# Teque5/caf_cookoff

Hardware: NVIDIA B200
Metric: CAF cells/s (400x8192 fp64 surface + peak) (higher is better)
Workload: dtype f64

## Files before the change

### caf_cookoff_b200/csrc/caf_kernels.cuh

```cuda
#pragma once
#include <cstdint>
#include <type_traits>
#include "fft16.cuh"

namespace caf {

constexpr int kThreads = 512;
constexpr int kL0 = 4096;
constexpr int kM = 8192;

enum Mode : int {
    kSurface = 0,
    kSpectrumHalf = 1,
    kSpectrumFull = 2,
    kXcorFull = 3,
    kXcorHalf = 4
};

struct PeakOut {
    double value;
    double freq_hz;
    unsigned long long doppler_idx;
    unsigned long long delay_idx;
};

template <typename T>
struct RowArgs {
    const cx<T>* in;
    const cx<T>* in2;
    cx<T>* hperm;
    const double* freqs;
    void* out;
    T* row_peak_val;
    unsigned long long* row_peak_idx;
    PeakOut* peak;
    unsigned long long* peak_words;
    unsigned long long row_offset;
    unsigned int* peak_seq;
    unsigned int seq_val;
    unsigned int* done_counter;
    unsigned int done_last;
    const cx<T>* tw1;
    const cx<T>* tw2;
    const cx<T>* g;
    double dt;
    int L;
    int D;
    int P;
    cx<T>* hshare;
    unsigned int* hflag;
    unsigned int epoch;
    int hprod1;
    const uint4* pull_src;
    uint4* pull_dst;
    unsigned int pull_n16;
    unsigned int* pull_counter;
    unsigned int pull_target;
    unsigned int flags;
    long long* trace;
};

template <typename T> struct Fab;
template <> struct Fab<double> {
    using E = double;
    static constexpr int kRegion = 280;
    static constexpr int kPlane = 16 * kRegion;
    static constexpr int kPipe = 2 * kPlane;
    static __device__ __forceinline__ void st(E* p, int i, double2 v) { p[i] = v.x; p[kPlane + i] = v.y; }
    static __device__ __forceinline__ double2 ld(const E* p, int i) { return make_double2(p[i], p[kPlane + i]); }
};
template <> struct Fab<float> {
    using E = float2;
    static constexpr int kRegion = 256;
    static constexpr int kPipe = 16 * kRegion;
    static __device__ __forceinline__ void st(E* p, int i, float2 v) { p[i] = v; }
    static __device__ __forceinline__ float2 ld(const E* p, int i) { return p[i]; }
};

template <typename T>
struct SmemLayout {
    static constexpr size_t kS = sizeof(typename Fab<T>::E) * 2 * Fab<T>::kPipe;
    static constexpr size_t kPtab = sizeof(cx<T>) * 2 * 2 * 48;
    static constexpr size_t kRed = 16 * 8 + 16 * 8;
    static constexpr size_t kCand = 2 * 256 * (8 + 4);
    static constexpr size_t kMisc = 64;
    static constexpr size_t kNeedle = sizeof(T) * 2 * kL0;
    static constexpr size_t offPtab = kS, offRed = offPtab + kPtab, offCand = offRed + kRed, offMisc = offCand + kCand,
                            offNeedle = offMisc + kMisc;
    static constexpr size_t kTotalNoNeedle = offNeedle;
    static constexpr size_t kTotal = offNeedle + kNeedle;
};

template <typename T>
struct Ctx {
    static constexpr bool kPadded = std::is_same<T, double>::value;
    typename Fab<T>::E* Sr;
    cx<T>* ptab;
    uint32_t tm_A;
    uint32_t tm_B;
    uint32_t tm_g;
    int w, lane, r, h, t;
    int wb;
    int hs[2];
    int hr;
    long long* tr;

    __device__ __forceinline__ void init(unsigned char* smem_raw, int tid) {
        const int hw_warp = tid >> 5;
        lane = tid & 31; r = tid >> 8;
        h = (lane & 7) | ((lane >> 1) & 8);
        const int sub = (lane >> 3) & 1;
        w = 2 * (hw_warp & 7) + sub;
        t = 16 * w + h;
        wb = Fab<T>::kRegion * w;
        hs[0] = h ^ (sub << 3); hs[1] = hs[0] ^ 8;
        hr = h ^ (((sub ^ h) & 1) << 3);
        Sr = reinterpret_cast<typename Fab<T>::E*>(smem_raw) + r * Fab<T>::kPipe;
        ptab = nullptr; tm_A = tm_B = tm_g = 0; tr = nullptr;
    }
    __device__ __forceinline__ int ix_block(int k) const {
        if constexpr (kPadded) return k * Fab<T>::kRegion + (t ^ ((t & 16) >> 1));
        else return k * 256 + 16 * w + hs[k & 1];
    }
    __device__ __forceinline__ int ix_own(int i) const {
        if constexpr (kPadded) return wb + 16 * i + (h ^ ((i & 1) << 3));
        else return wb + 16 * i + hs[i & 1];
    }
    __device__ __forceinline__ int ix_tw(int k) const {
        if constexpr (kPadded) return wb + 17 * k + h;
        else return wb + 16 * k + (hs[k & 1] ^ k);
    }
    __device__ __forceinline__ int ix_tr(int m) const {
        if constexpr (kPadded) return wb + 17 * h + m;
        else return wb + 16 * h + (m ^ hr);
    }
};

#ifdef CAF_TRACE
#define CAF_TR(c_, slot_) do { if ((c_).tr && (c_).lane == 0) (c_).tr[slot_] = clock64(); } while (0)
#else
#define CAF_TR(c_, slot_) do { } while (0)
#endif

__device__ __forceinline__ void tmem_ld_x16(uint32_t taddr, uint32_t (&r)[16]) {
    asm volatile("tcgen05.ld.sync.aligned.32x32b.x16.b32 {%0,%1,%2,%3,%4,%5,%6,%7,%8,%9,%10,%11,%12,%13,%14,%15}, [%16];\n"
                 : "=r"(r[0]), "=r"(r[1]), "=r"(r[2]), "=r"(r[3]), "=r"(r[4]), "=r"(r[5]), "=r"(r[6]), "=r"(r[7]),
                   "=r"(r[8]), "=r"(r[9]), "=r"(r[10]), "=r"(r[11]), "=r"(r[12]), "=r"(r[13]), "=r"(r[14]), "=r"(r[15])
                 : "r"(taddr) : "memory");
}
__device__ __forceinline__ void tmem_st_x16(uint32_t taddr, const uint32_t (&r)[16]) {
    asm volatile("tcgen05.st.sync.aligned.32x32b.x16.b32 [%0], {%1,%2,%3,%4,%5,%6,%7,%8,%9,%10,%11,%12,%13,%14,%15,%16};\n"
                 :: "r"(taddr), "r"(r[0]), "r"(r[1]), "r"(r[2]), "r"(r[3]), "r"(r[4]), "r"(r[5]), "r"(r[6]), "r"(r[7]),
                    "r"(r[8]), "r"(r[9]), "r"(r[10]), "r"(r[11]), "r"(r[12]), "r"(r[13]), "r"(r[14]), "r"(r[15]) : "memory");
}
__device__ __forceinline__ void tmem_ld_x8(uint32_t taddr, uint32_t (&r)[8]) {
    asm volatile("tcgen05.ld.sync.aligned.32x32b.x8.b32 {%0,%1,%2,%3,%4,%5,%6,%7}, [%8];\n"
                 : "=r"(r[0]), "=r"(r[1]), "=r"(r[2]), "=r"(r[3]), "=r"(r[4]), "=r"(r[5]), "=r"(r[6]), "=r"(r[7])
                 : "r"(taddr) : "memory");
}
__device__ __forceinline__ void tmem_st_x8(uint32_t taddr, const uint32_t (&r)[8]) {
    asm volatile("tcgen05.st.sync.aligned.32x32b.x8.b32 [%0], {%1,%2,%3,%4,%5,%6,%7,%8};\n"
                 :: "r"(taddr), "r"(r[0]), "r"(r[1]), "r"(r[2]), "r"(r[3]), "r"(r[4]), "r"(r[5]), "r"(r[6]), "r"(r[7]) : "memory");
}
__device__ __forceinline__ void tmem_wait_ld() { asm volatile("tcgen05.wait::ld.sync.aligned;\n" ::: "memory"); }
__device__ __forceinline__ void tmem_wait_st() { asm volatile("tcgen05.wait::st.sync.aligned;\n" ::: "memory"); }

__device__ __forceinline__ void tmem_ld_x4(uint32_t taddr, uint32_t (&r)[4]) {
    asm volatile("tcgen05.ld.sync.aligned.32x32b.x4.b32 {%0,%1,%2,%3}, [%4];\n"
                 : "=r"(r[0]), "=r"(r[1]), "=r"(r[2]), "=r"(r[3]) : "r"(taddr) : "memory");
}
__device__ __forceinline__ void tmem_st_x4(uint32_t taddr, const uint32_t (&r)[4]) {
    asm volatile("tcgen05.st.sync.aligned.32x32b.x4.b32 [%0], {%1,%2,%3,%4};\n"
                 :: "r"(taddr), "r"(r[0]), "r"(r[1]), "r"(r[2]), "r"(r[3]) : "memory");
}
__device__ __forceinline__ void tmem_ld_x2(uint32_t taddr, uint32_t (&r)[2]) {
    asm volatile("tcgen05.ld.sync.aligned.32x32b.x2.b32 {%0,%1}, [%2];\n" : "=r"(r[0]), "=r"(r[1]) : "r"(taddr) : "memory");
}
__device__ __forceinline__ void tmem_st_x2(uint32_t taddr, const uint32_t (&r)[2]) {
    asm volatile("tcgen05.st.sync.aligned.32x32b.x2.b32 [%0], {%1,%2};\n" :: "r"(taddr), "r"(r[0]), "r"(r[1]) : "memory");
}

template <typename T> struct TmemGeom;
template <> struct TmemGeom<double> { static constexpr int kColsPerC = 4, kAlloc = 512; };
template <> struct TmemGeom<float>  { static constexpr int kColsPerC = 2, kAlloc = 256; };

struct Raw4d { uint32_t r[16]; };
struct Raw4f { uint32_t r[8]; };
template <typename T> struct raw4_of;
template <> struct raw4_of<double> { using type = Raw4d; };
template <> struct raw4_of<float>  { using type = Raw4f; };
__device__ __forceinline__ void tmem_ld4_issue(uint32_t taddr, Raw4d& q) { tmem_ld_x16(taddr, q.r); }
__device__ __forceinline__ void tmem_ld4_issue(uint32_t taddr, Raw4f& q) { tmem_ld_x8(taddr, q.r); }
__device__ __forceinline__ void tmem_unpack4(const Raw4d& q, double2 (&o)[4]) {
#pragma unroll
    for (int i = 0; i < 4; ++i) {
        o[i].x = __hiloint2double((int)q.r[4 * i + 1], (int)q.r[4 * i]);
        o[i].y = __hiloint2double((int)q.r[4 * i + 3], (int)q.r[4 * i + 2]);
    }
}
__device__ __forceinline__ void tmem_unpack4(const Raw4f& q, float2 (&o)[4]) {
#pragma unroll
    for (int i = 0; i < 4; ++i) { o[i].x = __uint_as_float(q.r[2 * i]); o[i].y = __uint_as_float(q.r[2 * i + 1]); }
}
__device__ __forceinline__ void tmem_st4(uint32_t taddr, const double2 (&v)[4]) {
    uint32_t r[16];
#pragma unroll
    for (int i = 0; i < 4; ++i) {
        r[4 * i] = (uint32_t)__double2loint(v[i].x); r[4 * i + 1] = (uint32_t)__double2hiint(v[i].x);
        r[4 * i + 2] = (uint32_t)__double2loint(v[i].y); r[4 * i + 3] = (uint32_t)__double2hiint(v[i].y);
    }
    tmem_st_x16(taddr, r);
}
__device__ __forceinline__ void tmem_st4(uint32_t taddr, const float2 (&v)[4]) {
    uint32_t r[8];
#pragma unroll
    for (int i = 0; i < 4; ++i) { r[2 * i] = __float_as_uint(v[i].x); r[2 * i + 1] = __float_as_uint(v[i].y); }
    tmem_st_x8(taddr, r);
}

__device__ __forceinline__ double2 tmem_ld1(uint32_t taddr, double) {
    uint32_t r[4];
    tmem_ld_x4(taddr, r);
    tmem_wait_ld();
    return make_double2(__hiloint2double((int)r[1], (int)r[0]), __hiloint2double((int)r[3], (int)r[2]));
}
__device__ __forceinline__ float2 tmem_ld1(uint32_t taddr, float) {
    uint32_t r[2];
    tmem_ld_x2(taddr, r);
    tmem_wait_ld();
    return make_float2(__uint_as_float(r[0]), __uint_as_float(r[1]));
}
__device__ __forceinline__ void tmem_st1(uint32_t taddr, double2 v) {
    uint32_t r[4] = {(uint32_t)__double2loint(v.x), (uint32_t)__double2hiint(v.x), (uint32_t)__double2loint(v.y), (uint32_t)__double2hiint(v.y)};
    tmem_st_x4(taddr, r);
}
__device__ __forceinline__ void tmem_st1(uint32_t taddr, float2 v) {
    uint32_t r[2] = {__float_as_uint(v.x), __float_as_uint(v.y)};
    tmem_st_x2(taddr, r);
}

template <typename T>
__device__ __forceinline__ cx<T> ldg(const cx<T>* p) { return __ldg(p); }

__device__ __forceinline__ double2 unit_phasor(double n, double phi, double exact_sub) {
    double hi = n * phi;
    double lo = fma(n, phi, -hi);
    double fr = (hi - rint(hi)) + lo - exact_sub;
    fr -= rint(fr);
    double s, c;
    sincospi(2.0 * fr, &s, &c);
    return make_double2(c, s);
}

__device__ __forceinline__ void bar_group(int r) { asm volatile("bar.sync %0, 256;\n" :: "r"(r + 1) : "memory"); }

__device__ __forceinline__ void mbar_init(uint64_t* mb, int count) {
    asm volatile("mbarrier.init.shared::cta.b64 [%0], %1;\n" :: "r"((uint32_t)__cvta_generic_to_shared(mb)), "r"(count) : "memory");
}
__device__ __forceinline__ void mbar_arrive(uint64_t* mb) {
    asm volatile("{\n.reg .b64 st;\nmbarrier.arrive.shared::cta.b64 st, [%0];\n}\n"
                 :: "r"((uint32_t)__cvta_generic_to_shared(mb)) : "memory");
}
__device__ __forceinline__ void mbar_wait(uint64_t* mb, int parity) {
    const uint32_t addr = (uint32_t)__cvta_generic_to_shared(mb);
    asm volatile("{\n.reg .pred p;\nWAIT_%=:\nmbarrier.try_wait.parity.shared::cta.b64 p, [%0], %1;\n@p bra DONE_%=;\nbra WAIT_%=;\nDONE_%=:\n}\n"
                 :: "r"(addr), "r"(parity) : "memory");
}

template <typename T>
__device__ __forceinline__ void tmem_store_power_table(uint32_t taddr, cx<T> w) {
    constexpr int kC = TmemGeom<T>::kColsPerC;
    const cx<T> w2 = csq(w), w4 = csq(w2);
    cx<T> q[4];
    q[0] = mk<T>((T)1, (T)0); q[1] = w4; q[2] = csq(w4); q[3] = cmul(q[2], w4);
    tmem_st4(taddr, q);
    q[0] = w; q[1] = cmul(q[0], w4); q[2] = cmul(q[1], w4); q[3] = cmul(q[2], w4);
    tmem_st4(taddr + 4 * kC, q);
    q[0] = w2; q[1] = cmul(q[0], w4); q[2] = cmul(q[1], w4); q[3] = cmul(q[2], w4);
    tmem_st4(taddr + 8 * kC, q);
    q[0] = cmul(w2, w); q[1] = cmul(q[0], w4); q[2] = cmul(q[1], w4); q[3] = cmul(q[2], w4);
    tmem_st4(taddr + 12 * kC, q);
}

template <typename T, bool INV, int MODE, bool Q0_ONE>
__device__ __forceinline__ void fft16_in_tmem(cx<T> (&v)[16], uint32_t taddr) {
    constexpr int kC = TmemGeom<T>::kColsPerC;
    typename raw4_of<T>::type r0, r1, r2, r3;
    cx<T> q[4];
    tmem_ld4_issue(taddr, r0);
    tmem_wait_ld();
    tmem_ld4_issue(taddr + 4 * kC, r1);
    tmem_unpack4(r0, q);
    radix4_in<T, INV, MODE, Q0_ONE>(v[0], v[4], v[8], v[12], q[0], q[1], q[2], q[3]);
    tmem_wait_ld();
    tmem_ld4_issue(taddr + 8 * kC, r2);
    tmem_unpack4(r1, q);
    radix4_in<T, INV, MODE, false>(v[1], v[5], v[9], v[13], q[0], q[1], q[2], q[3]);
    tmem_wait_ld();
    tmem_ld4_issue(taddr + 12 * kC, r3);
    tmem_unpack4(r2, q);
    radix4_in<T, INV, MODE, false>(v[2], v[6], v[10], v[14], q[0], q[1], q[2], q[3]);
    tmem_wait_ld();
    tmem_unpack4(r3, q);
    radix4_in<T, INV, MODE, false>(v[3], v[7], v[11], v[15], q[0], q[1], q[2], q[3]);
    fft16_stage_b<T, INV>(v);
}

template <typename T, int MODE>
__device__ __forceinline__ void mul_table_tmem(cx<T> (&v)[16], uint32_t taddr) {
    constexpr int kC = TmemGeom<T>::kColsPerC;
    typename raw4_of<T>::type r0, r1, r2, r3;
    cx<T> q[4];
    tmem_ld4_issue(taddr, r0);
    tmem_ld4_issue(taddr + 4 * kC, r1);
    tmem_wait_ld();
    tmem_ld4_issue(taddr + 8 * kC, r2);
    tmem_ld4_issue(taddr + 12 * kC, r3);
    tmem_unpack4(r0, q);
#pragma unroll
    for (int a = 1; a < 4; ++a) v[4 * a] = tw_apply<MODE>(v[4 * a], q[a]);
    tmem_unpack4(r1, q);
#pragma unroll
    for (int a = 0; a < 4; ++a) v[1 + 4 * a] = tw_apply<MODE>(v[1 + 4 * a], q[a]);
    tmem_wait_ld();
    tmem_unpack4(r2, q);
#pragma unroll
    for (int a = 0; a < 4; ++a) v[2 + 4 * a] = tw_apply<MODE>(v[2 + 4 * a], q[a]);
    tmem_unpack4(r3, q);
#pragma unroll
    for (int a = 0; a < 4; ++a) v[3 + 4 * a] = tw_apply<MODE>(v[3 + 4 * a], q[a]);
}

template <typename T, typename Hook, typename Hook3>
__device__ __forceinline__ void forward_tail(cx<T> (&v)[16], const Ctx<T>& c,
                                             uint64_t* empty_mb, int empty_parity, Hook&& hook, Hook3&& hook3) {
    mul_table_tmem<T, kTwMul>(v, c.tm_A);
    CAF_TR(c, 3);
    if (empty_mb) mbar_wait(empty_mb, empty_parity);
    hook();
    bar_group(c.r);
#pragma unroll
    for (int k = 0; k < 16; ++k) Fab<T>::st(c.Sr, c.ix_block(k), v[k]);
    CAF_TR(c, 4);
    bar_group(c.r);
#pragma unroll
    for (int i = 0; i < 16; ++i) v[i] = Fab<T>::ld(c.Sr, c.ix_own(i));
    CAF_TR(c, 5);

    fft16<T, false>(v);
    CAF_TR(c, 6);
    __syncwarp();
#pragma unroll
    for (int k = 0; k < 16; ++k) Fab<T>::st(c.Sr, c.ix_tw(k), v[k]);
    __syncwarp();
#pragma unroll
    for (int m = 0; m < 16; ++m) v[m] = Fab<T>::ld(c.Sr, c.ix_tr(m));
    hook3();
    CAF_TR(c, 7);

    fft16_in_tmem<T, false, kTwMul, true>(v, c.tm_B);
    CAF_TR(c, 8);
}
template <typename T, typename Hook, typename Hook3>
__device__ __forceinline__ void forward_4096(cx<T> (&v)[16], const Ctx<T>& c,
                                             uint64_t* empty_mb, int empty_parity, Hook&& hook, Hook3&& hook3) {
    fft16<T, false>(v);
    forward_tail<T>(v, c, empty_mb, empty_parity, hook, hook3);
}

template <typename T, bool HFUSED>
__device__ __forceinline__ void inverse_4096(cx<T> (&v)[16], const Ctx<T>& c, uint32_t tm_h) {
    if constexpr (HFUSED) fft16_in_tmem<T, true, kTwConjX, false>(v, tm_h);
    else fft16<T, true>(v);
    CAF_TR(c, 10);
    __syncwarp();
#pragma unroll
    for (int k = 0; k < 16; ++k) Fab<T>::st(c.Sr, c.ix_tw(k), v[k]);
    __syncwarp();
#pragma unroll
    for (int m = 0; m < 16; ++m) v[m] = Fab<T>::ld(c.Sr, c.ix_tr(m));
    CAF_TR(c, 11);

    fft16_in_tmem<T, true, kTwMulConj, true>(v, c.tm_B);
    CAF_TR(c, 12);
    __syncwarp();
#pragma unroll
    for (int k = 0; k < 16; ++k) Fab<T>::st(c.Sr, c.ix_own(k), v[k]);
    CAF_TR(c, 13);
    bar_group(c.r);
#pragma unroll
    for (int k = 0; k < 16; ++k) v[k] = Fab<T>::ld(c.Sr, c.ix_block(k));
    CAF_TR(c, 14);

    fft16_in_tmem<T, true, kTwMulConj, true>(v, c.tm_A);
    CAF_TR(c, 15);
}

template <typename T, int J>
__device__ __forceinline__ cx<T> mul_w32_inv(cx<T> a) {
    constexpr T Cc[8] = {(T)1.0L, (T)0.98078528040323044913L, (T)0.92387953251128675613L, (T)0.83146961230254523708L,
                         (T)0.70710678118654752440L, (T)0.55557023301960222474L, (T)0.38268343236508977173L,
                         (T)0.19509032201612826785L};
    constexpr T Ss[8] = {(T)0.0L, (T)0.19509032201612826785L, (T)0.38268343236508977173L, (T)0.55557023301960222474L,
                         (T)0.70710678118654752440L, (T)0.83146961230254523708L, (T)0.92387953251128675613L,
                         (T)0.98078528040323044913L};
    if constexpr (J == 0) return a;
    else if constexpr (J == 8) return mk<T>(-a.y, a.x);
    else if constexpr (J < 8) return mk<T>(a.x * Cc[J] - a.y * Ss[J], a.x * Ss[J] + a.y * Cc[J]);
    else return mk<T>(-a.x * Ss[J - 8] - a.y * Cc[J - 8], a.x * Cc[J - 8] - a.y * Ss[J - 8]);
}

__device__ __forceinline__ void pack_peak_words(const PeakOut& p, unsigned long long global_row_offset,
                                                unsigned long long* __restrict__ words) {
    words[0] = (unsigned long long)__double_as_longlong(p.value);
    words[1] = (p.doppler_idx == ~0ull) ? ~0ull : p.doppler_idx + global_row_offset;
    words[2] = p.delay_idx;
    words[3] = (unsigned long long)__double_as_longlong(p.freq_hz);
}

template <typename T>
__device__ __forceinline__ void amax_take(T& best, int& bidx, T m, int k) {
    if (m > best || (m == best && k < bidx)) { best = m; bidx = k; }
}

template <int I> using ic = std::integral_constant<int, I>;

template <typename T, int MODE, bool FULL, bool SHARED = false>
__global__ void __launch_bounds__(kThreads, 1) caf_rows_kernel(const RowArgs<T> a) {
    using C = cx<T>;
    using SL = SmemLayout<T>;
    using TG = TmemGeom<T>;
    extern __shared__ __align__(16) unsigned char smem_raw[];
    C* ptab = reinterpret_cast<C*>(smem_raw + SL::offPtab);
    unsigned long long* red_idx = reinterpret_cast<unsigned long long*>(smem_raw + SL::offRed);
    double* red_val = reinterpret_cast<double*>(smem_raw + SL::offRed + 128);
    double* cand_val = reinterpret_cast<double*>(smem_raw + SL::offCand);
    int* cand_idx = reinterpret_cast<int*>(smem_raw + SL::offCand + 2 * 256 * 8);
    uint32_t* misc = reinterpret_cast<uint32_t*>(smem_raw + SL::offMisc);
    uint64_t* mb_full = reinterpret_cast<uint64_t*>(smem_raw + SL::offMisc + 16);
    uint64_t* mb_empty = reinterpret_cast<uint64_t*>(smem_raw + SL::offMisc + 24);

    const int tid = threadIdx.x;
#ifdef CAF_TRACE
    long long tr_g0 = 0, tr_c0 = clock64();
    asm volatile("mov.u64 %0, %%globaltimer;" : "=l"(tr_g0));
#endif
    Ctx<T> c;
    const int hw_warp = tid >> 5;
    c.init(smem_raw, tid);
    c.ptab = ptab;
    const int w = c.w, lane = c.lane, r = c.r, h = c.h, t = c.t, tg = tid & 255, wg = hw_warp & 7;

    constexpr bool kHalfZero = (MODE == kSurface || MODE == kSpectrumHalf || MODE == kXcorHalf);
    constexpr bool kWritesH = (MODE == kSpectrumHalf || MODE == kSpectrumFull);
    constexpr bool kUseTmem = (MODE == kSurface);
    T* const ndl_re = reinterpret_cast<T*>(smem_raw + SL::offNeedle);
    T* const ndl_im = ndl_re + kL0;

    const int rows_per_pair = (MODE == kSurface) ? a.D : 1;
    const long long n_items = (long long)a.P * rows_per_pair;
    const int lo = (int)(n_items * blockIdx.x / gridDim.x), hi = (int)(n_items * (blockIdx.x + 1) / gridDim.x);
    int pair = lo / rows_per_pair, row = lo - pair * rows_per_pair;

    int buf = 0;
    int cur_pair = -1;
    int posts = 0;
    bool drain_pending = false;
    bool h_from_share = false;
    C v[16];

    if constexpr (MODE == kSurface) asm volatile("griddepcontrol.launch_dependents;\n" ::: "memory");
    const C tb0 = ldg<T>(a.tw1 + 256 + t), tb1 = ldg<T>(a.tw2 + 16 + h), tb4 = ldg<T>(a.g + t);
    bool preloaded = false;
    double phi_first = 0.0;
    if constexpr (MODE == kSurface) {
        if (lo < hi) {
            const bool producer0 = !SHARED || (int)blockIdx.x == ((r == 0) ? 0 : a.hprod1);
            const C* src = (producer0 ? a.in2 : a.in) + (long long)pair * a.L;
#pragma unroll
            for (int q = 0; q < (int)sizeof(C) / 8; ++q) {
                const long long byte0 = ((long long)tg + 256 * q) * 128;
                if (byte0 < (long long)a.L * (long long)sizeof(C))
                    asm volatile("prefetch.global.L2 [%0];\n" :: "l"(reinterpret_cast<const char*>(src) + byte0));
            }
            if (tg == 255) asm volatile("prefetch.global.L2 [%0];\n" :: "l"(a.freqs + row));
        }
    }

    uint4 pulled = make_uint4(0u, 0u, 0u, 0u);
    const unsigned int pull_i = blockIdx.x * 64u + (unsigned int)(tid - 448);
    if constexpr (MODE == kSurface && SHARED) {
        if (a.pull_src != nullptr && tid >= 448 && pull_i < a.pull_n16)
            asm volatile("ld.volatile.global.v4.u32 {%0,%1,%2,%3}, [%4];\n"
                         : "=r"(pulled.x), "=r"(pulled.y), "=r"(pulled.z), "=r"(pulled.w) : "l"(a.pull_src + pull_i) : "memory");
    }

    if (tid == 0) {
        mbar_init(mb_full, 256);
        mbar_init(mb_empty, 256);
        asm volatile("fence.mbarrier_init.release.cluster;\n" ::: "memory");
    }

    uint32_t tm_h = 0;
    {
        if (hw_warp == 0) {
            asm volatile("tcgen05.alloc.cta_group::1.sync.aligned.shared::cta.b32 [%0], %1;\n"
                         :: "l"((uint64_t)__cvta_generic_to_shared(&misc[0])), "n"(TG::kAlloc));
            asm volatile("tcgen05.relinquish_alloc_permit.cta_group::1.sync.aligned;\n");
        }
        asm volatile("tcgen05.fence::before_thread_sync;\n");
        __syncthreads();
        asm volatile("tcgen05.fence::after_thread_sync;\n");
        const uint32_t base = misc[0] + ((uint32_t)(32 * (hw_warp & 3)) << 16);
        const int j = hw_warp >> 2;
        tm_h = base + (uint32_t)((16 * j) * TG::kColsPerC);
        c.tm_A = base + (uint32_t)((64 + 16 * (j & 1)) * TG::kColsPerC);
        c.tm_B = base + (uint32_t)(96 * TG::kColsPerC);
        c.tm_g = base + (uint32_t)((112 + 4 * j) * TG::kColsPerC);
        if (r == 0) tmem_store_power_table<T>(c.tm_A, tb0);
        else if (j == 2) tmem_store_power_table<T>(c.tm_B, tb1);
        tmem_st1(c.tm_g, tb4);
        tmem_wait_st();
        asm volatile("tcgen05.fence::before_thread_sync;\n");
        __syncthreads();
        asm volatile("tcgen05.fence::after_thread_sync;\n");
    }

    if constexpr (MODE == kSurface) {
        if (!(SHARED && (a.flags & 1u))) asm volatile("griddepcontrol.wait;\n" ::: "memory");
        if constexpr (SHARED) {
            if (a.pull_src != nullptr) {
                if (tid >= 448) {
                    unsigned int i = pull_i;
                    if (i < a.pull_n16) __stcg(a.pull_dst + i, pulled);
                    for (i += gridDim.x * 64u; i < a.pull_n16; i += gridDim.x * 64u) {
                        uint4 q;
                        asm volatile("ld.volatile.global.v4.u32 {%0,%1,%2,%3}, [%4];\n"
                                     : "=r"(q.x), "=r"(q.y), "=r"(q.z), "=r"(q.w) : "l"(a.pull_src + i) : "memory");
                        __stcg(a.pull_dst + i, q);
                    }
                    __threadfence();
                    __syncwarp();
                    if (lane == 0) asm volatile("red.release.gpu.global.add.u32 [%0], 1;\n" :: "l"(a.pull_counter) : "memory");
                }
                if (tid == 0) {
                    unsigned int seen;
                    do {
                        asm volatile("ld.acquire.gpu.global.u32 %0, [%1];\n" : "=r"(seen) : "l"(a.pull_counter) : "memory");
                    } while ((int)(seen - a.pull_target) < 0);
                }
                __syncthreads();
            }
        }
        if (lo < hi) {
            const bool producer0 = !SHARED || (int)blockIdx.x == ((r == 0) ? 0 : a.hprod1);
            const C* src = (producer0 ? a.in2 : a.in) + (long long)pair * a.L;
#pragma unroll
            for (int i = 0; i < 16; ++i) {
                const int n = t + 256 * i;
                v[i] = (n < a.L) ? (SHARED ? __ldcg(src + n) : ldg<T>(src + n)) : mk<T>((T)0, (T)0);
            }
            preloaded = true;
            phi_first = (SHARED ? __ldcg(a.freqs + row) : __ldg(a.freqs + row)) * a.dt;
        }
    }

    auto fill_ptab = [&](int buf, double phi) {
        if (tg < 48) {
            const int e = tg, which = e >> 4, idx = e & 15;
            const int n = idx << (which == 0 ? 8 : which == 1 ? 4 : 0);
            double2 p = unit_phasor((double)n, phi, (double)(r * n) * (1.0 / 8192.0));
            ptab[(buf * 2 + r) * 48 + e] = mk<T>((T)p.x, (T)p.y);
        }
    };
    auto fill_ptab_both = [&](int buf, double phi) {
        if (tg < 96) {
            const int rr = tg >= 48, e = tg - 48 * rr, which = e >> 4, idx = e & 15;
            const int n = idx << (which == 0 ? 8 : which == 1 ? 4 : 0);
            double2 p = unit_phasor((double)n, phi, (double)(rr * n) * (1.0 / 8192.0));
            ptab[(buf * 2 + rr) * 48 + e] = mk<T>((T)p.x, (T)p.y);
        }
    };
    auto phasor_fft16 = [&](C (&v)[16], int buf) {
        const C* pt = ptab + (buf * 2 + r) * 48;
        const C s4 = pt[4];
        const C base = cmul(pt[16 + w], pt[32 + h]);
        {
            const C q1 = cmul(base, s4), q2 = cmul(q1, s4), q3 = cmul(q2, s4);
            radix4_in<T, false, kTwMul, false>(v[0], v[4], v[8], v[12], base, q1, q2, q3);
        }
#pragma unroll
        for (int cc = 1; cc < 4; ++cc) {
            const C q0 = cmul(base, pt[cc]), q1 = cmul(q0, s4), q2 = cmul(q1, s4), q3 = cmul(q2, s4);
            radix4_in<T, false, kTwMul, false>(v[cc], v[cc + 4], v[cc + 8], v[cc + 12], q0, q1, q2, q3);
        }
        fft16_stage_b<T, false>(v);
    };
    auto load_half = [&](C (&v)[16], const C* src, int L) {
#pragma unroll
        for (int i = 0; i < 16; ++i) {
            const int n = t + 256 * i;
            v[i] = (n < L) ? ldg<T>(src + n) : mk<T>((T)0, (T)0);
        }
    };


    auto fold_candidates = [&](int slot, int it) {
        double bv = 0.0;
        int bi = 0x7fffffff;
#pragma unroll
        for (int q = 0; q < 8; ++q) {
            const double cv = cand_val[slot * 256 + lane + 32 * q];
            const int ci = cand_idx[slot * 256 + lane + 32 * q];
            amax_take<double>(bv, bi, cv, ci);
        }
#pragma unroll
        for (int off = 16; off > 0; off >>= 1) {
            double ov = __shfl_xor_sync(0xffffffffu, bv, off);
            int oi = __shfl_xor_sync(0xffffffffu, bi, off);
            amax_take<double>(bv, bi, ov, oi);
        }
        if (lane == 0) {
            if (!(bv > 0.0)) bi = 0;
            if (a.row_peak_val) a.row_peak_val[it] = (T)bv;
            if (a.row_peak_idx) a.row_peak_idx[it] = (unsigned long long)bi;
        }
    };

    auto empty_gate = [&](uint64_t*& mb, int& par) {
        if (r == 1 && drain_pending) { mb = mb_empty; par = (posts - 1) & 1; drain_pending = false; }
        else { mb = nullptr; par = 0; }
    };

    c.tr = nullptr;
    for (int item = lo; item < hi; ++item, buf ^= 1) {
#ifdef CAF_TRACE
        c.tr = (a.trace && item - lo < 8) ? a.trace + ((((long long)blockIdx.x * 16 + hw_warp) * 8 + (item - lo)) * 32) : nullptr;
#endif
        CAF_TR(c, 0);
        if constexpr (MODE == kSurface) {
            if (pair != cur_pair) {
                cur_pair = pair;
                constexpr bool shared_h = SHARED;
                const int my_prod_cta = (r == 0) ? 0 : a.hprod1;
                const bool producer = !shared_h || (int)blockIdx.x == my_prod_cta;
                const bool park = shared_h && a.hprod1 != 0 && ((int)blockIdx.x == 0 || (int)blockIdx.x == a.hprod1);
                bar_group(r);
                if (producer) {
                    fill_ptab(buf, 0.0);
                    if (!preloaded) load_half(v, a.in2 + (long long)pair * a.L, a.L);
                    preloaded = false;
                }
                bar_group(r);
                if (producer) {
#ifdef CAF_TRACE
                    long long* tr_row = c.tr;
                    if (a.trace && item == lo) c.tr = a.trace + ((((long long)blockIdx.x * 16 + hw_warp) * 8 + 7) * 32);
#endif
                    CAF_TR(c, 0);
                    phasor_fft16(v, buf);
                    uint64_t* mb; int par;
                    empty_gate(mb, par);
                    forward_tail<T>(v, c, mb, par, [&] {
                                        if (r == 1 && mb != nullptr && wg == 3) fold_candidates((buf ^ 1) & 1, item - 1);
                                    }, []{});
                    const T sc = (T)(1.0 / 8192.0);
#pragma unroll
                    for (int q = 0; q < 4; ++q) {
                        C tmp[4];
#pragma unroll
                        for (int i = 0; i < 4; ++i) {
                            tmp[i] = mk<T>(v[q + 4 * i].x * sc, v[q + 4 * i].y * sc);
                            if (shared_h) __stcg(a.hshare + (q + 4 * i) * kThreads + tid, tmp[i]);
                        }
                        tmem_st4(tm_h + 4 * q * TG::kColsPerC, tmp);
                    }
                    if (shared_h) {
                        __threadfence();
                        bar_group(r);
                        if (tg == 0) asm volatile("st.release.gpu.global.u32 [%0], %1;\n" :: "l"(a.hflag + r), "r"(a.epoch) : "memory");
                    }
                    CAF_TR(c, 9);
#ifdef CAF_TRACE
                    c.tr = tr_row;
#endif
                } else {
                    h_from_share = true;
                }
                if (park) __syncthreads();
                if (!preloaded) load_half(v, a.in + (long long)pair * a.L, a.L);
                const bool first_row_phi = preloaded || (item == lo);
                preloaded = false;
                __syncthreads();
                {
                    T* const dst = (r == 0) ? ndl_re : ndl_im;
#pragma unroll
                    for (int i = 0; i < 16; ++i) dst[t + 256 * i] = (r == 0) ? v[i].x : v[i].y;
                }
                fill_ptab(buf, first_row_phi ? phi_first : a.freqs[row] * a.dt);
                __syncthreads();
            }
            CAF_TR(c, 1);
#pragma unroll
            for (int i = 0; i < 16; ++i) v[i] = mk<T>(ndl_re[t + 256 * i], ndl_im[t + 256 * i]);
            phasor_fft16(v, buf);
            CAF_TR(c, 2);
        } else if constexpr (kHalfZero) {
            bar_group(r);
            fill_ptab(buf, 0.0);
            load_half(v, a.in + (long long)pair * a.L, a.L);
            bar_group(r);
            phasor_fft16(v, buf);
        } else {
            const C* src = a.in + (long long)pair * kM;
#pragma unroll
            for (int i = 0; i < 16; ++i) {
                const int n = t + 256 * i;
                C x0 = ldg<T>(src + n), x1 = ldg<T>(src + n + kL0);
                if (r == 0) v[i] = cadd(x0, x1);
                else v[i] = cmulc(csub(x0, x1), ldg<T>(a.g + n));
            }
            fft16<T, false>(v);
        }

        {
            uint64_t* mb; int par;
            empty_gate(mb, par);
            const bool had_mail = (mb != nullptr);
            forward_tail<T>(v, c, mb, par, [&] {
                                    if constexpr (MODE == kSurface) {
                                        if (r == 1) {
                                            if ((item + 1 < hi) && (row + 1 < a.D)) fill_ptab_both(buf ^ 1, a.freqs[row + 1] * a.dt);
                                            if (had_mail && wg == 3) fold_candidates((buf ^ 1) & 1, item - 1);
                                        }
                                    }
                                },
                                [&] {
                                    if constexpr (kUseTmem) {
                                        if (SHARED && h_from_share && lane == 0) {
                                            unsigned int seen;
                                            do {
                                                asm volatile("ld.acquire.gpu.global.u32 %0, [%1];\n" : "=r"(seen) : "l"(a.hflag + r) : "memory");
                                            } while ((int)(seen - a.epoch) < 0);
                                        }
                                    }
                                });
        }

        C* hp = a.hperm + (long long)pair * kM;
        if constexpr (kWritesH) {
            const T sc = (T)(1.0 / 8192.0);
#pragma unroll
            for (int k = 0; k < 16; ++k) hp[((k * 16 + w) * 2 + r) * 16 + h] = mk<T>(v[k].x * sc, v[k].y * sc);
        } else {
            if constexpr (kUseTmem) {
                if (SHARED && h_from_share) {
                    h_from_share = false;
                    __syncwarp();
#pragma unroll
                    for (int k = 0; k < 16; ++k) Fab<T>::st(c.Sr, c.ix_own(k), v[k]);
#pragma unroll
                    for (int k = 0; k < 16; ++k) v[k] = __ldcg(a.hshare + k * kThreads + tid);
#pragma unroll
                    for (int q = 0; q < 4; ++q) {
                        C hv[4];
#pragma unroll
                        for (int i = 0; i < 4; ++i) hv[i] = v[q + 4 * i];
                        tmem_st4(tm_h + 4 * q * TG::kColsPerC, hv);
                    }
#pragma unroll
                    for (int k = 0; k < 16; ++k) v[k] = Fab<T>::ld(c.Sr, c.ix_own(k));
                    tmem_wait_st();
                }
                CAF_TR(c, 9);
                inverse_4096<T, true>(v, c, tm_h);
            } else {
#pragma unroll
                for (int k = 0; k < 16; ++k) v[k] = cmulc(ldg<T>(hp + ((k * 16 + w) * 2 + r) * 16 + h), v[k]);
                CAF_TR(c, 9);
                inverse_4096<T, false>(v, c, 0u);
            }

            if (r == 1) {
                const C gt = tmem_ld1(c.tm_g, T());
                auto post = [&](auto jt) {
                    constexpr int j = decltype(jt)::value;
                    v[j] = cmul(v[j], mul_w32_inv<T, j>(gt));
                };
                post(ic<0>{}); post(ic<1>{}); post(ic<2>{}); post(ic<3>{}); post(ic<4>{}); post(ic<5>{}); post(ic<6>{}); post(ic<7>{});
                post(ic<8>{}); post(ic<9>{}); post(ic<10>{}); post(ic<11>{}); post(ic<12>{}); post(ic<13>{}); post(ic<14>{}); post(ic<15>{});
                CAF_TR(c, 16);
                bar_group(1);
#pragma unroll
                for (int k = 0; k < 16; ++k) Fab<T>::st(c.Sr, c.ix_block(k), v[k]);
                mbar_arrive(mb_full);
                CAF_TR(c, 17);
                ++posts;
                drain_pending = true;

            } else {
                const int L = FULL ? kL0 : a.L;
                const int nout = 2 * L, skip = kM - nout;
                T* orow = (MODE == kSurface && a.out) ? reinterpret_cast<T*>(a.out) + item * (long long)nout : nullptr;
                C* ocx = (MODE != kSurface) ? reinterpret_cast<C*>(a.out) + (long long)pair * kM : nullptr;
                T best0 = (T)0, best1 = (T)0;
                int bidx0 = 0, bidx1 = 0;
                auto emit = [&](C y, int kp, T& best, int& bidx) {
                    if constexpr (MODE == kSurface) {
                        const T m = y.x * y.x + y.y * y.y;
                        if constexpr (FULL) {
                            if (orow) orow[kp] = m;
                            if (m > best) { best = m; bidx = kp; }
                        } else {
                            int k = -1;
                            if (kp <= L) k = kp; else if (kp > kM - L) k = kp - skip;
                            if (k >= 0 && k < nout) {
                                if (orow) orow[k] = m;
                                if (m > best) { best = m; bidx = k; }
                            }
                        }
                    } else {
                        ocx[kp] = y;
                    }
                };
                CAF_TR(c, 16);
                mbar_wait(mb_full, posts & 1);
                CAF_TR(c, 17);
                const typename Fab<T>::E* mail = c.Sr + Fab<T>::kPipe;
#pragma unroll
                for (int k = 0; k < 16; ++k) {
                    const C Bp = Fab<T>::ld(mail, c.ix_block(k));
                    const int n = t + 256 * k;
                    emit(cadd(v[k], Bp), n, best0, bidx0);
                    emit(csub(v[k], Bp), n + kL0, best1, bidx1);
                }
                if constexpr (MODE == kSurface) {
                    T best = best0;
                    int bidx = bidx0;
                    if (best1 > best) { best = best1; bidx = bidx1; }
                    cand_val[(buf & 1) * 256 + tg] = (double)best;
                    cand_idx[(buf & 1) * 256 + tg] = bidx;
                }
                mbar_arrive(mb_empty);
                CAF_TR(c, 18);
                ++posts;
            }
        }
        CAF_TR(c, 19);
        if (++row == rows_per_pair) { row = 0; ++pair; }
    }
    if constexpr (MODE == kSurface) {
        if (r == 1 && drain_pending) {
            mbar_wait(mb_empty, (posts - 1) & 1);
            if (wg == 3) fold_candidates((buf ^ 1) & 1, hi - 1);
        }
    }

    {
        asm volatile("tcgen05.fence::before_thread_sync;\n");
        __syncthreads();
        if (hw_warp == 0) {
            asm volatile("tcgen05.dealloc.cta_group::1.sync.aligned.b32 %0, %1;\n" :: "r"(misc[0]), "n"(TG::kAlloc));
        }
    }

#ifdef CAF_TRACE
    if (a.trace && (tid & 31) == 0) {
        long long g1; asm volatile("mov.u64 %0, %%globaltimer;" : "=l"(g1));
        long long* q = a.trace + (((long long)blockIdx.x * 16 + hw_warp) * 8 + 0) * 32;
        q[20] = tr_g0; q[21] = g1; q[22] = tr_c0; q[23] = clock64();
    }
#endif
    if constexpr (MODE == kSurface) {
        if (SHARED && a.peak != nullptr && a.done_counter != nullptr && r == 1 && wg == 3) {
            unsigned int last = 0;
            if (lane == 0) {
                __threadfence();
                last = (atomicAdd(a.done_counter, 1u) == a.done_last) ? 1u : 0u;
            }
            last = __shfl_sync(0xffffffffu, last, 0);
            if (last) {
                __threadfence();
                double best = 0.0;
                int brow = 0x7fffffff;
                for (int d0 = 0; d0 < a.D; d0 += 128) {
                    double vv[4];
#pragma unroll
                    for (int q = 0; q < 4; ++q) {
                        const int d = d0 + 32 * q + lane;
                        vv[q] = (d < a.D) ? (double)__ldcg(a.row_peak_val + d) : 0.0;
                    }
#pragma unroll
                    for (int q = 0; q < 4; ++q)
                        if (vv[q] > best) { best = vv[q]; brow = d0 + 32 * q + lane; }
                }
#pragma unroll
                for (int off = 16; off > 0; off >>= 1) {
                    double ov = __shfl_xor_sync(0xffffffffu, best, off);
                    int oi = __shfl_xor_sync(0xffffffffu, brow, off);
                    amax_take<double>(best, brow, ov, oi);
                }
                if (lane == 0) {
                    PeakOut p;
                    if (best > 0.0 && brow != 0x7fffffff) {
                        p.value = best; p.freq_hz = a.freqs[brow];
                        p.doppler_idx = (unsigned long long)brow; p.delay_idx = __ldcg(a.row_peak_idx + brow);
                    } else {
                        p.value = 0.0; p.freq_hz = 0.0; p.doppler_idx = ~0ull; p.delay_idx = 0;
                    }
                    *a.peak = p;
                    if (a.peak_words) pack_peak_words(p, a.row_offset, a.peak_words);
                    if (a.peak_seq) {
                        __threadfence_system();
                        *reinterpret_cast<volatile unsigned int*>(a.peak_seq) = a.seq_val;
                    }
                }
            }
        }
    }
#ifdef CAF_TRACE
    if (a.trace && tid == 0) {
        long long g2; asm volatile("mov.u64 %0, %%globaltimer;" : "=l"(g2));
        a.trace[(((long long)blockIdx.x * 16 + 0) * 8 + 0) * 32 + 29] = g2;
    }
#endif
}

template <typename T>
__global__ void __launch_bounds__(256) caf_peak_kernel(const T* __restrict__ row_val,
                                                       const unsigned long long* __restrict__ row_idx,
                                                       const double* __restrict__ freqs, int D, PeakOut* out,
                                                       unsigned long long* words = nullptr,
                                                       unsigned long long row_offset = 0ull) {
    __shared__ double sv[8];
    __shared__ int si[8];
    const long long base = (long long)blockIdx.x * D;
    double best = 0.0;
    int brow = 0x7fffffff;
    for (int d = threadIdx.x; d < D; d += blockDim.x) {
        double v = (double)row_val[base + d];
        if (v > best) { best = v; brow = d; }
    }
#pragma unroll
    for (int off = 16; off > 0; off >>= 1) {
        double ov = __shfl_xor_sync(0xffffffffu, best, off);
        int oi = __shfl_xor_sync(0xffffffffu, brow, off);
        amax_take<double>(best, brow, ov, oi);
    }
    if ((threadIdx.x & 31) == 0) { sv[threadIdx.x >> 5] = best; si[threadIdx.x >> 5] = brow; }
    __syncthreads();
    if (threadIdx.x == 0) {
        for (int q = 1; q < 8; ++q) amax_take<double>(best, brow, sv[q], si[q]);
        PeakOut p;
        if (best > 0.0 && brow != 0x7fffffff) {
            p.value = best; p.freq_hz = freqs[brow];
            p.doppler_idx = (unsigned long long)brow; p.delay_idx = row_idx[base + brow];
        } else {
            p.value = 0.0; p.freq_hz = 0.0; p.doppler_idx = ~0ull; p.delay_idx = 0;
        }
        if (out) out[blockIdx.x] = p;
        if (words && blockIdx.x == 0) pack_peak_words(p, row_offset, words);
    }
}

__global__ void caf_peak_pack_kernel(const PeakOut* __restrict__ local, unsigned long long global_row_offset,
                                     unsigned long long* __restrict__ words) {
    if (threadIdx.x == 0) {
        PeakOut p;
        if (local) p = *local;
        else { p.value = 0.0; p.freq_hz = 0.0; p.doppler_idx = ~0ull; p.delay_idx = 0; }
        pack_peak_words(p, global_row_offset, words);
    }
}

constexpr unsigned long long kPeakNone = ~0ull, kPeakRemoteError = ~0ull - 1ull;
__global__ void caf_peak_resolve_kernel(const unsigned long long* __restrict__ words, int world, PeakOut* out,
                                        int* __restrict__ status) {
    if (threadIdx.x != 0) return;
    PeakOut best; best.value = 0.0; best.freq_hz = 0.0; best.doppler_idx = ~0ull; best.delay_idx = 0;
    int st = 0;
    for (int r = 0; r < world; ++r) {
        const unsigned long long* w = words + 4 * r;
        if (w[1] == kPeakRemoteError) { st = 1; continue; }
        if (w[1] == kPeakNone) continue;
        const double v = __longlong_as_double((long long)w[0]);
        if (v > best.value || (v == best.value && v > 0.0 && w[1] < best.doppler_idx)) {
            best.value = v; best.freq_hz = __longlong_as_double((long long)w[3]); best.doppler_idx = w[1]; best.delay_idx = w[2];
        }
    }
    *out = best;
    if (status) *status = st;
}

__global__ void caf_peak_exchange_kernel(const unsigned long long* __restrict__ send, unsigned long long* const* __restrict__ peer_mail,
                                         unsigned long long* mail, int world, int rank, unsigned long long epoch,
                                         PeakOut* out, int* __restrict__ status) {
    const int lane = threadIdx.x;
    const size_t par = (size_t)(epoch & 1ull);
    const unsigned long long w0 = send[0], w1 = send[1], w2 = send[2], w3 = send[3];
    for (int s = lane; s < world; s += 32) {
        unsigned long long* dst = peer_mail[s] + (par * world + rank) * 8;
        asm volatile("st.volatile.global.v2.u64 [%0], {%1, %2};\n" :: "l"(dst), "l"(w0), "l"(w1) : "memory");
        asm volatile("st.volatile.global.v2.u64 [%0], {%1, %2};\n" :: "l"(dst + 2), "l"(w2), "l"(w3) : "memory");
        __threadfence_system();
        asm volatile("st.release.sys.global.u64 [%0], %1;\n" :: "l"(dst + 4), "l"(epoch) : "memory");
    }
    double bv = 0.0, bf = 0.0;
    unsigned long long brow = ~0ull, bdel = 0ull;
    int st = 0;
    for (int s = lane; s < world; s += 32) {
        const unsigned long long* src = mail + (par * world + s) * 8;
        unsigned long long tag = 0ull;
        unsigned int polls = 0;
        for (;;) {
            asm volatile("ld.acquire.sys.global.u64 %0, [%1];\n" : "=l"(tag) : "l"(src + 4) : "memory");
            if (tag == epoch) break;
            if (++polls == (1u << 27)) { st = 1; break; }
        }
        if (tag != epoch) continue;
        unsigned long long r0, r1, r2, r3;
        asm volatile("ld.volatile.global.v2.u64 {%0, %1}, [%2];\n" : "=l"(r0), "=l"(r1) : "l"(src) : "memory");
        asm volatile("ld.volatile.global.v2.u64 {%0, %1}, [%2];\n" : "=l"(r2), "=l"(r3) : "l"(src + 2) : "memory");
        if (r1 == kPeakRemoteError) { st = 1; continue; }
        if (r1 == kPeakNone) continue;
        const double v = __longlong_as_double((long long)r0);
        if (v > bv || (v == bv && v > 0.0 && r1 < brow)) { bv = v; bf = __longlong_as_double((long long)r3); brow = r1; bdel = r2; }
    }
#pragma unroll
    for (int off = 16; off > 0; off >>= 1) {
        const double ov = __shfl_xor_sync(0xffffffffu, bv, off), of = __shfl_xor_sync(0xffffffffu, bf, off);
        const unsigned long long orow = __shfl_xor_sync(0xffffffffu, brow, off), odel = __shfl_xor_sync(0xffffffffu, bdel, off);
        st |= __shfl_xor_sync(0xffffffffu, st, off);
        if (ov > bv || (ov == bv && ov > 0.0 && orow < brow)) { bv = ov; bf = of; brow = orow; bdel = odel; }
    }
    if (lane == 0) {
        PeakOut best; best.value = bv; best.freq_hz = bf; best.doppler_idx = brow; best.delay_idx = bdel;
        *out = best;
        if (status) *status = st;
    }
}

template <typename T>
__global__ void __launch_bounds__(256) caf_layout_kernel(const T* __restrict__ rust, T* __restrict__ out, int L, int W,
                                                         int lag0, T* __restrict__ row_val,
                                                         unsigned long long* __restrict__ row_idx) {
    __shared__ double sv[8];
    __shared__ int si[8];
    const long long row = blockIdx.x;
    const T* src = rust + row * 2LL * L;
    T* dst = out + row * (long long)W;
    double best = 0.0;
    int bidx = 0x7fffffff;
    for (int j = threadIdx.x; j < W; j += blockDim.x) {
        int k = lag0 - j;
        if (k < 0) k += 2 * L;
        const T m = sqrt(src[k]);
        dst[j] = m;
        if ((double)m > best) { best = (double)m; bidx = j; }
    }
#pragma unroll
    for (int off = 16; off > 0; off >>= 1) {
        double ov = __shfl_xor_sync(0xffffffffu, best, off);
        int oi = __shfl_xor_sync(0xffffffffu, bidx, off);
        amax_take<double>(best, bidx, ov, oi);
    }
    if ((threadIdx.x & 31) == 0) { sv[threadIdx.x >> 5] = best; si[threadIdx.x >> 5] = bidx; }
    __syncthreads();
    if (threadIdx.x == 0) {
        for (int q = 1; q < 8; ++q) amax_take<double>(best, bidx, sv[q], si[q]);
        if (!(best > 0.0)) bidx = 0;
        row_val[row] = (T)best;
        row_idx[row] = (unsigned long long)bidx;
    }
}

template <typename T>
__global__ void caf_apply_shift_kernel(const cx<T>* __restrict__ in, cx<T>* __restrict__ out, long long n,
                                       double phi ) {
    for (long long i = blockIdx.x * (long long)blockDim.x + threadIdx.x; i < n;
         i += (long long)gridDim.x * blockDim.x) {
        double2 p = unit_phasor((double)i, phi, 0.0);
        cx<T> x = in[i];
        out[i] = mk<T>((T)((double)x.x * p.x - (double)x.y * p.y), (T)((double)x.x * p.y + (double)x.y * p.x));
    }
}

__global__ void caf_widen_c64_kernel(const float2* __restrict__ in, double2* __restrict__ out, long long n) {
    for (long long i = blockIdx.x * (long long)blockDim.x + threadIdx.x; i < n; i += (long long)gridDim.x * blockDim.x) {
        const float2 x = in[i];
        out[i] = make_double2((double)x.x, (double)x.y);
    }
}

template <typename T>
__global__ void caf_fold_circular_kernel(const cx<T>* __restrict__ y, cx<T>* __restrict__ out, int n, int big_n) {
    int k = blockIdx.x * blockDim.x + threadIdx.x;
    if (k < n) {
        cx<T> a = y[k];
        cx<T> b = (k == 0) ? mk<T>((T)0, (T)0) : y[big_n - n + k];
        out[k] = cadd(a, b);
    }
}

template <typename T>
__global__ void __launch_bounds__(512) caf_fma_probe_kernel(T* sink, int iters, T seed) {
    T a0 = seed + (T)threadIdx.x, a1 = a0 + (T)1, a2 = a0 + (T)2, a3 = a0 + (T)3;
    T a4 = a0 + (T)4, a5 = a0 + (T)5, a6 = a0 + (T)6, a7 = a0 + (T)7;
    const T m = (T)0.999999, c = (T)1e-6;
    for (int i = 0; i < iters; ++i) {
#pragma unroll
        for (int u = 0; u < 8; ++u) {
            a0 = fma(a0, m, c); a1 = fma(a1, m, c); a2 = fma(a2, m, c); a3 = fma(a3, m, c);
            a4 = fma(a4, m, c); a5 = fma(a5, m, c); a6 = fma(a6, m, c); a7 = fma(a7, m, c);
        }
    }
    T r = ((a0 + a1) + (a2 + a3)) + ((a4 + a5) + (a6 + a7));
    if (r == (T)123456789) sink[0] = r;
}

}
```

Baseline: 95.34 billion.

## Split final butterfly and emit symmetrically across both thread groups

The final inverse-FFT butterfly exchange used to be lopsided: group 1 posted all 16 values and group 0 did all the combine, magnitude, store and argmax work. Now each group posts half its values, waits on the other group's mailbox, and then combines and emits 8 outputs pairs itself. Per-group candidate buffers and paired full/empty mbarriers make this work, and candidate folding moves from the forward hook to after the emit on the chore group. The aim is to balance the epilogue and cut idle time, at the cost of more shared memory and a two-way barrier handshake per row.

```diff
diff --git a/caf_cookoff_b200/csrc/caf_kernels.cuh b/caf_cookoff_b200/csrc/caf_kernels.cuh
--- a/caf_cookoff_b200/csrc/caf_kernels.cuh
+++ b/caf_cookoff_b200/csrc/caf_kernels.cuh
@@ -85,10 +85,10 @@
     static constexpr size_t kCand = 2 * 256 * (8 + 4);
     static constexpr size_t kMisc = 64;
     static constexpr size_t kNeedle = sizeof(T) * 2 * kL0;
-    static constexpr size_t offPtab = kS, offRed = offPtab + kPtab, offCand = offRed + kRed, offMisc = offCand + kCand,
-                            offNeedle = offMisc + kMisc;
+    static constexpr size_t offPtab = kS, offRed = offPtab + kPtab, offCand0 = offRed + kRed, offMisc = offCand0 + kCand,
+                            offNeedle = offMisc + kMisc, offCand1 = offNeedle + kNeedle;
     static constexpr size_t kTotalNoNeedle = offNeedle;
-    static constexpr size_t kTotal = offNeedle + kNeedle;
+    static constexpr size_t kTotal = offCand1 + kCand;
 };
 
 template <typename T>
@@ -337,7 +337,9 @@
     mul_table_tmem<T, kTwMul>(v, c.tm_A);
     CAF_TR(c, 3);
     if (empty_mb) mbar_wait(empty_mb, empty_parity);
+    CAF_TR(c, 24);
     hook();
+    CAF_TR(c, 25);
     bar_group(c.r);
 #pragma unroll
     for (int k = 0; k < 16; ++k) Fab<T>::st(c.Sr, c.ix_block(k), v[k]);
@@ -434,11 +436,11 @@
     C* ptab = reinterpret_cast<C*>(smem_raw + SL::offPtab);
     unsigned long long* red_idx = reinterpret_cast<unsigned long long*>(smem_raw + SL::offRed);
     double* red_val = reinterpret_cast<double*>(smem_raw + SL::offRed + 128);
-    double* cand_val = reinterpret_cast<double*>(smem_raw + SL::offCand);
-    int* cand_idx = reinterpret_cast<int*>(smem_raw + SL::offCand + 2 * 256 * 8);
+    auto cand_val = [&](int g) { return reinterpret_cast<double*>(smem_raw + (g ? SL::offCand1 : SL::offCand0)); };
+    auto cand_idx = [&](int g) { return reinterpret_cast<int*>(smem_raw + (g ? SL::offCand1 : SL::offCand0) + 2 * 256 * 8); };
     uint32_t* misc = reinterpret_cast<uint32_t*>(smem_raw + SL::offMisc);
     uint64_t* mb_full = reinterpret_cast<uint64_t*>(smem_raw + SL::offMisc + 16);
-    uint64_t* mb_empty = reinterpret_cast<uint64_t*>(smem_raw + SL::offMisc + 24);
+    uint64_t* mb_empty = reinterpret_cast<uint64_t*>(smem_raw + SL::offMisc + 32);
 
     const int tid = threadIdx.x;
 #ifdef CAF_TRACE
@@ -462,10 +464,8 @@
     const int lo = (int)(n_items * blockIdx.x / gridDim.x), hi = (int)(n_items * (blockIdx.x + 1) / gridDim.x);
     int pair = lo / rows_per_pair, row = lo - pair * rows_per_pair;
 
-    int buf = 0;
     int cur_pair = -1;
     int posts = 0;
-    bool drain_pending = false;
     bool h_from_share = false;
     C v[16];
 
@@ -496,8 +496,10 @@
     }
 
     if (tid == 0) {
-        mbar_init(mb_full, 256);
-        mbar_init(mb_empty, 256);
+        for (int g = 0; g < 2; ++g) {
+            mbar_init(mb_full + g, 256);
+            mbar_init(mb_empty + g, 256);
+        }
         asm volatile("fence.mbarrier_init.release.cluster;\n" ::: "memory");
     }
 
@@ -605,14 +607,19 @@
     };
 
 
+    constexpr int kChore = 1;
+    const bool chore = (r == kChore);
     auto fold_candidates = [&](int slot, int it) {
         double bv = 0.0;
         int bi = 0x7fffffff;
-#pragma unroll
-        for (int q = 0; q < 8; ++q) {
-            const double cv = cand_val[slot * 256 + lane + 32 * q];
-            const int ci = cand_idx[slot * 256 + lane + 32 * q];
-            amax_take<double>(bv, bi, cv, ci);
+#pragma unroll 1
+        for (int g = 0; g < 2; ++g) {
+#pragma unroll
+            for (int q = 0; q < 8; ++q) {
+                const double cv = cand_val(g)[slot * 256 + lane + 32 * q];
+                const int ci = cand_idx(g)[slot * 256 + lane + 32 * q];
+                amax_take<double>(bv, bi, cv, ci);
+            }
         }
 #pragma unroll
         for (int off = 16; off > 0; off >>= 1) {
@@ -628,12 +635,13 @@
     };
 
     auto empty_gate = [&](uint64_t*& mb, int& par) {
-        if (r == 1 && drain_pending) { mb = mb_empty; par = (posts - 1) & 1; drain_pending = false; }
+        if (posts > 0) { mb = mb_empty + r; par = (posts - 1) & 1; }
         else { mb = nullptr; par = 0; }
     };
 
     c.tr = nullptr;
-    for (int item = lo; item < hi; ++item, buf ^= 1) {
+    for (int item = lo; item < hi; ++item) {
+        const int buf = item & 1;
 #ifdef CAF_TRACE
         c.tr = (a.trace && item - lo < 8) ? a.trace + ((((long long)blockIdx.x * 16 + hw_warp) * 8 + (item - lo)) * 32) : nullptr;
 #endif
@@ -661,9 +669,7 @@
                     phasor_fft16(v, buf);
                     uint64_t* mb; int par;
                     empty_gate(mb, par);
-                    forward_tail<T>(v, c, mb, par, [&] {
-                                        if (r == 1 && mb != nullptr && wg == 3) fold_candidates((buf ^ 1) & 1, item - 1);
-                                    }, []{});
+                    forward_tail<T>(v, c, mb, par, []{}, []{});
                     const T sc = (T)(1.0 / 8192.0);
 #pragma unroll
                     for (int q = 0; q < 4; ++q) {
@@ -726,13 +732,9 @@
         {
             uint64_t* mb; int par;
             empty_gate(mb, par);
-            const bool had_mail = (mb != nullptr);
             forward_tail<T>(v, c, mb, par, [&] {
                                     if constexpr (MODE == kSurface) {
-                                        if (r == 1) {
-                                            if ((item + 1 < hi) && (row + 1 < a.D)) fill_ptab_both(buf ^ 1, a.freqs[row + 1] * a.dt);
-                                            if (had_mail && wg == 3) fold_candidates((buf ^ 1) & 1, item - 1);
-                                        }
+                                        if (chore && (item + 1 < hi) && (row + 1 < a.D)) fill_ptab_both(buf ^ 1, a.freqs[row + 1] * a.dt);
                                     }
                                 },
                                 [&] {
@@ -781,79 +783,80 @@
                 inverse_4096<T, false>(v, c, 0u);
             }
 
-            if (r == 1) {
-                const C gt = tmem_ld1(c.tm_g, T());
-                auto post = [&](auto jt) {
-                    constexpr int j = decltype(jt)::value;
-                    v[j] = cmul(v[j], mul_w32_inv<T, j>(gt));
-                };
-                post(ic<0>{}); post(ic<1>{}); post(ic<2>{}); post(ic<3>{}); post(ic<4>{}); post(ic<5>{}); post(ic<6>{}); post(ic<7>{});
-                post(ic<8>{}); post(ic<9>{}); post(ic<10>{}); post(ic<11>{}); post(ic<12>{}); post(ic<13>{}); post(ic<14>{}); post(ic<15>{});
+            auto emit = [&](C y, int kp, T& best, int& bidx, T* orow, C* ocx, int L) {
+                const int nout = 2 * L, skip = kM - nout;
+                if constexpr (MODE == kSurface) {
+                    const T m = y.x * y.x + y.y * y.y;
+                    if constexpr (FULL) {
+                        if (orow) orow[kp] = m;
+                        if (m > best) { best = m; bidx = kp; }
+                    } else {
+                        int k = -1;
+                        if (kp <= L) k = kp; else if (kp > kM - L) k = kp - skip;
+                        if (k >= 0 && k < nout) {
+                            if (orow) orow[k] = m;
+                            if (m > best) { best = m; bidx = k; }
+                        }
+                    }
+                } else {
+                    ocx[kp] = y;
+                }
+            };
+            auto exchange_and_finish = [&](auto rt) {
+                constexpr int R = decltype(rt)::value;
+                constexpr int kOwn = 8 * R, kPost = 8 - kOwn;
+                if constexpr (R == 1) {
+                    const C gt = tmem_ld1(c.tm_g, T());
+                    auto twiddle = [&](auto jt) {
+                        constexpr int j = decltype(jt)::value;
+                        v[j] = cmul(v[j], mul_w32_inv<T, j>(gt));
+                    };
+                    twiddle(ic<0>{}); twiddle(ic<1>{}); twiddle(ic<2>{}); twiddle(ic<3>{});
+                    twiddle(ic<4>{}); twiddle(ic<5>{}); twiddle(ic<6>{}); twiddle(ic<7>{});
+                    twiddle(ic<8>{}); twiddle(ic<9>{}); twiddle(ic<10>{}); twiddle(ic<11>{});
+                    twiddle(ic<12>{}); twiddle(ic<13>{}); twiddle(ic<14>{}); twiddle(ic<15>{});
+                }
                 CAF_TR(c, 16);
-                bar_group(1);
-#pragma unroll
-                for (int k = 0; k < 16; ++k) Fab<T>::st(c.Sr, c.ix_block(k), v[k]);
-                mbar_arrive(mb_full);
+                bar_group(R);
+#pragma unroll
+                for (int j = 0; j < 8; ++j) Fab<T>::st(c.Sr, c.ix_block(kPost + j), v[kPost + j]);
+                mbar_arrive(mb_full + R);
+                mbar_wait(mb_full + (1 - R), posts & 1);
+                const typename Fab<T>::E* mail = c.Sr + (R == 0 ? Fab<T>::kPipe : -Fab<T>::kPipe);
+#pragma unroll
+                for (int j = 0; j < 8; ++j) v[kPost + j] = Fab<T>::ld(mail, c.ix_block(kOwn + j));
+                mbar_arrive(mb_empty + (1 - R));
                 CAF_TR(c, 17);
                 ++posts;
-                drain_pending = true;
-
-            } else {
-                const int L = FULL ? kL0 : a.L;
-                const int nout = 2 * L, skip = kM - nout;
-                T* orow = (MODE == kSurface && a.out) ? reinterpret_cast<T*>(a.out) + item * (long long)nout : nullptr;
-                C* ocx = (MODE != kSurface) ? reinterpret_cast<C*>(a.out) + (long long)pair * kM : nullptr;
                 T best0 = (T)0, best1 = (T)0;
                 int bidx0 = 0, bidx1 = 0;
-                auto emit = [&](C y, int kp, T& best, int& bidx) {
-                    if constexpr (MODE == kSurface) {
-                        const T m = y.x * y.x + y.y * y.y;
-                        if constexpr (FULL) {
-                            if (orow) orow[kp] = m;
-                            if (m > best) { best = m; bidx = kp; }
-                        } else {
-                            int k = -1;
-                            if (kp <= L) k = kp; else if (kp > kM - L) k = kp - skip;
-                            if (k >= 0 && k < nout) {
-                                if (orow) orow[k] = m;
-                                if (m > best) { best = m; bidx = k; }
-                            }
-                        }
-                    } else {
-                        ocx[kp] = y;
-                    }
-                };
-                CAF_TR(c, 16);
-                mbar_wait(mb_full, posts & 1);
-                CAF_TR(c, 17);
-                const typename Fab<T>::E* mail = c.Sr + Fab<T>::kPipe;
-#pragma unroll
-                for (int k = 0; k < 16; ++k) {
-                    const C Bp = Fab<T>::ld(mail, c.ix_block(k));
-                    const int n = t + 256 * k;
-                    emit(cadd(v[k], Bp), n, best0, bidx0);
-                    emit(csub(v[k], Bp), n + kL0, best1, bidx1);
+                const int L = FULL ? kL0 : a.L;
+                T* orow = (MODE == kSurface && a.out) ? reinterpret_cast<T*>(a.out) + item * (long long)(2 * L) : nullptr;
+                C* ocx = (MODE != kSurface) ? reinterpret_cast<C*>(a.out) + (long long)pair * kM : nullptr;
+#pragma unroll
+                for (int j = 0; j < 8; ++j) {
+                    const C A = (R == 0) ? v[j] : v[kPost + j], Bp = (R == 0) ? v[kPost + j] : v[kOwn + j];
+                    const int n = t + 256 * (kOwn + j);
+                    emit(cadd(A, Bp), n, best0, bidx0, orow, ocx, L);
+                    emit(csub(A, Bp), n + kL0, best1, bidx1, orow, ocx, L);
                 }
                 if constexpr (MODE == kSurface) {
                     T best = best0;
                     int bidx = bidx0;
                     if (best1 > best) { best = best1; bidx = bidx1; }
-                    cand_val[(buf & 1) * 256 + tg] = (double)best;
-                    cand_idx[(buf & 1) * 256 + tg] = bidx;
-                }
-                mbar_arrive(mb_empty);
+                    cand_val(R)[buf * 256 + tg] = (double)best;
+                    cand_idx(R)[buf * 256 + tg] = bidx;
+                }
                 CAF_TR(c, 18);
-                ++posts;
-            }
+                if constexpr (MODE == kSurface && R == kChore) {
+                    if (wg == 3 && posts >= 2) fold_candidates(buf ^ 1, item - 1);
+                }
+            };
+            if (r == 0) exchange_and_finish(ic<0>{});
+            else exchange_and_finish(ic<1>{});
         }
         CAF_TR(c, 19);
         if (++row == rows_per_pair) { row = 0; ++pair; }
-    }
-    if constexpr (MODE == kSurface) {
-        if (r == 1 && drain_pending) {
-            mbar_wait(mb_empty, (posts - 1) & 1);
-            if (wg == 3) fold_candidates((buf ^ 1) & 1, hi - 1);
-        }
     }
 
     {
@@ -863,6 +866,9 @@
             asm volatile("tcgen05.dealloc.cta_group::1.sync.aligned.b32 %0, %1;\n" :: "r"(misc[0]), "n"(TG::kAlloc));
         }
     }
+    if constexpr (MODE == kSurface) {
+        if (chore && wg == 3 && posts >= 1) fold_candidates((hi - 1) & 1, hi - 1);
+    }
 
 #ifdef CAF_TRACE
     if (a.trace && (tid & 31) == 0) {
@@ -872,7 +878,7 @@
     }
 #endif
     if constexpr (MODE == kSurface) {
-        if (SHARED && a.peak != nullptr && a.done_counter != nullptr && r == 1 && wg == 3) {
+        if (SHARED && a.peak != nullptr && a.done_counter != nullptr && chore && wg == 3) {
             unsigned int last = 0;
             if (lane == 0) {
                 __threadfence();
```

Result: slower. 88.03 billion (median of 6 runs) (-7.7%).
